# Layr-Labs/rust-kzg-bn254

Measured on AMD Instinct MI355X. Metric: G1-MSM (scalar,point) pairs/s = 2^20 x KZG coeff-form commitments/s, 2^20-point SRS, higher is better.
Workload: dtype int32x9 (29-bit limbs, 64-bit accumulate); 1 GPU; G1 MSM 2^20 scalars (KZG::commit_coeff_form), scalars resident in HBM; step k commits buffer k mod 8 (8 distinct resident scalar sets, 256 MiB); pipeline_depth=2, steps_per_launch=1

## Files before the change

### rust-kzg-bn254_amd/csrc/curve.h

```cpp
#pragma once
#include "field29.h"

#if !defined(__HIPCC__)
struct uint4 { uint32_t x, y, z, w; };
#endif

#if !defined(KZG_NO_MADD_PAIRED) && !defined(KZG_MADD_PAIRED)
#define KZG_MADD_PAIRED 1
#endif

namespace kzg {

struct Affine {
    Fq x, y;
};

struct Xyzz {
    Fq x, y, zz, zzz;
    bool inf;
};

KZG_HD void xyzz_set_inf(Xyzz& r) {
    fe_set_zero(r.x); fe_set_zero(r.y); fe_set_zero(r.zz); fe_set_zero(r.zzz);
    r.inf = true;
// ... 12 lines not shown
    Fq u, v, w, s, m, t, xx;
    fe_dbl(u, y2); fe_norm(u);
    fe_sqr(v, u);
    fe_mul(w, u, v);
    fe_mul(s, x2, v);
    fe_sqr(xx, x2);
    fe_add(m, xx, xx); fe_add(m, m, xx); fe_norm(m);
    fe_sqr(r.x, m);
    fe_sub(r.x, r.x, s); fe_sub(r.x, r.x, s); fe_norm(r.x);
    fe_sub(t, s, r.x);
    fe_mul(t, m, t);
    fe_mul(u, w, y2);
    fe_sub(r.y, t, u); fe_norm(r.y);
    r.zz = v;
    r.zzz = w;
    r.inf = false;
}

KZG_HD_NOINLINE void xyzz_dbl_affine(Xyzz& r, const Fq& x2, const Fq& y2) { xyzz_dbl_affine_impl(r, x2, y2); }

KZG_HD void xyzz_dbl_impl(Xyzz& r, const Xyzz& p) {
    if (p.inf) { r = p; return; }
    Fq u, v, w, s, m, t, xx;
    fe_dbl(u, p.y); fe_norm(u);
    fe_sqr(v, u);
    fe_mul(w, u, v);
    fe_mul(s, p.x, v);
    fe_sqr(xx, p.x);
    fe_add(m, xx, xx); fe_add(m, m, xx); fe_norm(m);
    Fq x3, y3;
    fe_sqr(x3, m);
    fe_sub(x3, x3, s); fe_sub(x3, x3, s); fe_norm(x3);
    fe_sub(t, s, x3);
    fe_mul(t, m, t);
    fe_mul(u, w, p.y);
    fe_sub(y3, t, u); fe_norm(y3);
    fe_mul(r.zz, v, p.zz);
    fe_mul(r.zzz, w, p.zzz);
    r.x = x3; r.y = y3; r.inf = false;
}

KZG_HD_NOINLINE void xyzz_dbl(Xyzz& r, const Xyzz& p) { xyzz_dbl_impl(r, p); }

template <bool INLINE_SLOW>
KZG_HD void xyzz_madd_exceptional(Xyzz& acc, const Fq& x2, const Fq& y2s, const Fq& rr) {
    if (fe_is_zero_mod(rr)) {
        if (INLINE_SLOW) xyzz_dbl_affine_impl(acc, x2, y2s);
        else xyzz_dbl_affine(acc, x2, y2s);
    } else {
        xyzz_set_inf(acc);
    }
}

template <bool INLINE_SLOW = false>
KZG_HD void xyzz_madd(Xyzz& acc, const Affine& p, uint32_t neg) {
    if (acc.inf) { xyzz_from_affine(acc, p, neg); return; }
    Fq y2s, u2, s2, pp_, rr_, P, R, ppp, q, t, v;
    fe_cneg(y2s, p.y, neg);
#if defined(KZG_MADD_PAIRED)
    fe_mul2(u2, p.x, acc.zz, s2, y2s, acc.zzz);
#else
    fe_mul(u2, p.x, acc.zz);
    fe_mul(s2, y2s, acc.zzz);
#endif
    fe_sub(P, u2, acc.x);
    fe_sub(R, s2, acc.y);
#if defined(KZG_MADD_PAIRED)
    fe_sqr2(pp_, P, rr_, R);
#else
    fe_sqr(pp_, P);
    fe_sqr(rr_, R);
#endif
    if (__builtin_expect(fe_is_zero_mod(pp_), 0)) { xyzz_madd_exceptional<INLINE_SLOW>(acc, p.x, y2s, rr_); return; }
#if defined(KZG_MADD_PAIRED)
    fe_mul2(ppp, P, pp_, q, acc.x, pp_);
#else
    fe_mul(ppp, P, pp_);
    fe_mul(q, acc.x, pp_);
#endif
    fe_sub(v, rr_, ppp); fe_sub(v, v, q); fe_sub(v, v, q); fe_norm(v);
    fe_sub(t, q, v);
    fe_mulsub(acc.y, R, t, acc.y, ppp);
    acc.x = v;
#if defined(KZG_MADD_PAIRED)
    { Fq z2, z3; fe_mul2(z2, acc.zz, pp_, z3, acc.zzz, ppp); acc.zz = z2; acc.zzz = z3; }
#else
    fe_mul(acc.zz, acc.zz, pp_);
    fe_mul(acc.zzz, acc.zzz, ppp);
#endif
}

template <bool INLINE_SLOW>
KZG_HD void xyzz_add_exceptional(Xyzz& r, const Xyzz& a, const Fq& rr) {
    if (fe_is_zero_mod(rr)) {
        if (INLINE_SLOW) xyzz_dbl_impl(r, a);
        else xyzz_dbl(r, a);
    } else {
        xyzz_set_inf(r);
    }
}

template <bool INLINE_SLOW = false>
KZG_HD void xyzz_add(Xyzz& r, const Xyzz& a, const Xyzz& b) {
    if (a.inf) { r = b; return; }
    if (b.inf) { r = a; return; }
    Fq u1, u2, s1, s2, P, R, pp_, rr_, ppp, q, t, v;
    fe_mul(u1, a.x, b.zz);
    fe_mul(u2, b.x, a.zz);
    fe_mul(s1, a.y, b.zzz);
    fe_mul(s2, b.y, a.zzz);
    fe_sub(P, u2, u1);
    fe_sub(R, s2, s1);
    fe_sqr(pp_, P);
    fe_sqr(rr_, R);
    if (__builtin_expect(fe_is_zero_mod(pp_), 0)) { xyzz_add_exceptional<INLINE_SLOW>(r, a, rr_); return; }
    fe_mul(ppp, P, pp_);
    fe_mul(q, u1, pp_);
    fe_sub(v, rr_, ppp); fe_sub(v, v, q); fe_sub(v, v, q); fe_norm(v);
    fe_sub(t, q, v);
    Fq y3;
    fe_mulsub(y3, R, t, s1, ppp);
    fe_mul(t, a.zz, b.zz);
    fe_mul(r.zz, t, pp_);
    fe_mul(t, a.zzz, b.zzz);
    fe_mul(r.zzz, t, ppp);
    r.x = v; r.y = y3; r.inf = false;
}

KZG_HD bool affine_load(Affine& p, const uint4* __restrict__ src) {
    uint4 a = src[0], b = src[1], c = src[2], d = src[3];
    uint32_t wx[8] = {a.x, a.y, a.z, a.w, b.x, b.y, b.z, b.w};
    uint32_t wy[8] = {c.x, c.y, c.z, c.w, d.x, d.y, d.z, d.w};
    fe_unpack(p.x, wx);
    fe_unpack(p.y, wy);
    uint32_t any = a.x | a.y | a.z | a.w | b.x | b.y | b.z | b.w | c.x | c.y | c.z | c.w | d.x | d.y | d.z | d.w;
    return any != 0;
}

KZG_HD void xyzz_store(int32_t* __restrict__ base, size_t stride, size_t i, const Xyzz& v) {
    const Fq* c[4] = {&v.x, &v.y, &v.zz, &v.zzz};
#pragma unroll
    for (int q = 0; q < 4; ++q)
#pragma unroll
        for (int j = 0; j < NL; ++j) base[(size_t)(q * NL + j) * stride + i] = v.inf ? 0 : c[q]->l[j];
}
KZG_HD void xyzz_load(Xyzz& v, const int32_t* __restrict__ base, size_t stride, size_t i) {
    Fq* c[4] = {&v.x, &v.y, &v.zz, &v.zzz};
#pragma unroll
    for (int q = 0; q < 4; ++q)
#pragma unroll
        for (int j = 0; j < NL; ++j) c[q]->l[j] = base[(size_t)(q * NL + j) * stride + i];
    v.inf = fe_is_literal_zero(v.zz);
}

KZG_HD void affine_wire_to_device(uint32_t out[16], const uint32_t in[16]) {
    Fq x, y;
    fe_from_wire(x, in);
    fe_from_wire(y, in + 8);
    fe_canon(x);
    fe_canon(y);
    fe_pack(out, x);
    fe_pack(out + 8, y);
}
KZG_HD void xyzz_to_wire(uint32_t out[32], const Xyzz& v) {
    if (v.inf) {
#pragma unroll
        for (int j = 0; j < 32; ++j) out[j] = 0;
        return;
    }
    fe_to_wire(out, v.x);
    fe_to_wire(out + 8, v.y);
    fe_to_wire(out + 16, v.zz);
    fe_to_wire(out + 24, v.zzz);
}

}
```

### rust-kzg-bn254_amd/csrc/engine.h

```cpp
#pragma once
#include <hip/hip_runtime.h>
#include <cstdint>
#include <functional>
#include <map>
#include <mutex>
#include <string>
#include "../../include/kzg_bn254_mi355x.h"

namespace kzg {

struct DeviceBuffer {
    void* p = nullptr;
    size_t bytes = 0;
    hipError_t reserve(size_t need) {
        if (need <= bytes) return hipSuccess;
        if (p) { hipError_t e = hipFree(p); p = nullptr; bytes = 0; if (e != hipSuccess) return e; }
        size_t cap = need + need / 8;
        hipError_t e = hipMalloc(&p, cap);
        if (e == hipSuccess) bytes = cap;
        return e;
    }
    void release() { if (p) { (void)hipFree(p); p = nullptr; bytes = 0; } }
    template <class T> T* as() const { return reinterpret_cast<T*>(p); }
};
// ... 58 lines not shown
#endif

struct kzg_ctx {
    int device = 0;
    hipStream_t stream = nullptr;
    std::mutex mu;
    std::string last_error;
    int msm_c_override = 0;
    int msm_seg_override = 0;
    int reduction_lanes = 0;
    bool profiling = false;
    bool lds_attr_set = false;
    bool poly_lds_attr_set = false;
    uint32_t acc_wave_slots = 3 * 1024;
    kzg::MsmWorkspace msm;
    kzg::MsmWorkspace msm_x[KZG_NUM_SLOTS - 1];
    hipStream_t stream_x[KZG_NUM_SLOTS - 1] = {};
    kzg::MsmPending* slot_pending[KZG_NUM_SLOTS] = {};
    kzg::NttWorkspace ntt;
    int32_t* ondomain_inv[13] = {};
    kzg::NttWorkspace ntt_x[KZG_NUM_SLOTS - 1];
    void* vb_pinned = nullptr;
    size_t vb_pinned_bytes = 0;
    kzg::DeviceBuffer rccl_buf;
    void* rccl_pinned = nullptr;
    size_t rccl_pinned_bytes = 0;
    kzg::PolySet poly[KZG_NUM_SLOTS];
    kzg::LagProof lag[KZG_NUM_SLOTS];
    hipStream_t lag_stream = nullptr;
    hipEvent_t lag_phase1[KZG_NUM_SLOTS] = {};
    hipEvent_t lag_uploaded[KZG_NUM_SLOTS] = {};
    kzg::MsmWorkspace& slot_msm(int slot) { return slot ? msm_x[slot - 1] : msm; }
    kzg::BlobStream* blob_stream = nullptr;
    hipEvent_t last_sorted = nullptr;
    hipStream_t last_sorted_stream = nullptr;
    kzg::NttWorkspace& slot_ntt(int slot) { return slot ? ntt_x[slot - 1] : ntt; }
    kzg::DeviceBuffer mp[6];
    kzg::NttWorkspace mp_ntt;
    kzg::DeviceBuffer mv[4];
    kzg::NttWorkspace mv_ntt;
};

struct kzg_srs {
    kzg_ctx* ctx = nullptr;
    mutable std::mutex lazy_mu;
    uint4* d_points = nullptr;
    size_t n = 0;
    int pre_c = 0;
    int pre_W = 0;
    uint4* d_small = nullptr;
    int small_c = 0;
    int small_W = 0;
    uint4* d_bits = nullptr;
    mutable uint4* d_t3 = nullptr;
    mutable uint32_t t3_n = 0;
    std::map<size_t, kzg_srs*> lagrange;
    size_t lagrange_of = 0;
    std::map<std::pair<size_t, size_t>, uint4*> multiproof;
};

namespace kzg {

struct MsmBases {
    const uint4* points = nullptr;
    uint32_t table_stride = 0;
    int c = 0;
    int W = 0;
    bool bitsum = false;
    bool naf = false;
};
constexpr int SRS_SMALL_C = 15;
constexpr size_t SRS_SMALL_MAX = (size_t)1 << 13;
constexpr size_t SRS_NAF_MIN = (size_t)1 << 11;
constexpr size_t MSM_NAF_MIN = (size_t)1 << 14;
inline int srs_naf_c(size_t n) {
    if (n < ((size_t)1 << 15)) return 13;
    return n >= ((size_t)1 << 20) ? 17 : n >= ((size_t)1 << 18) ? 16 : 15;
}
inline uint4* srs_bits(const kzg_srs* srs) { std::lock_guard<std::mutex> lk(srs->lazy_mu); return srs->d_bits; }
inline uint4* srs_t3(const kzg_srs* srs) { std::lock_guard<std::mutex> lk(srs->lazy_mu); return srs->d_t3; }
inline kzg_srs* srs_cached_lagrange(const kzg_srs* srs, size_t n) {
    std::lock_guard<std::mutex> lk(srs->lazy_mu);
    auto it = srs->lagrange.find(n);
    return it == srs->lagrange.end() ? nullptr : it->second;
}
inline MsmBases srs_bases(const kzg_srs* srs, size_t offset, size_t n, bool allow_tables) {
    MsmBases b;
    std::lock_guard<std::mutex> lk(srs->lazy_mu);
    b.points = srs->d_points + 4 * offset;
    if (allow_tables && srs->pre_W > 0) {
        b.table_stride = (uint32_t)srs->n; b.c = srs->pre_c; b.W = srs->pre_W;
        if (srs->d_small && n <= SRS_SMALL_MAX) { b.points = srs->d_small + 4 * offset; b.c = srs->small_c; b.W = srs->small_W; }
        if (srs->d_bits && n <= 4096) {
            b.points = srs->d_bits + 4 * offset; b.c = 0; b.W = 255; b.bitsum = true;
        }
        if (srs->d_bits && n >= MSM_NAF_MIN) {
            b.points = srs->d_bits + 4 * offset; b.c = srs_naf_c(n); b.W = 255; b.naf = true;
        }
    }
    return b;
}

int32_t msm_run(kzg_ctx* ctx, const MsmBases& bases, const void* d_scalars, size_t n,
                uint64_t out_xy[8], uint8_t* out_inf, uint64_t* out_xyzz);

int32_t msm_slot_stream(kzg_ctx* ctx, int slot, hipStream_t* out);
int32_t msm_begin(kzg_ctx* ctx, int slot, const MsmBases& bases, const void* d_scalars, size_t n);
int32_t msm_end(kzg_ctx* ctx, int slot, uint64_t out_xy[8], uint8_t* out_inf, uint64_t* out_xyzz);
void msm_drop_slots(kzg_ctx* ctx);
int32_t msm_run_batch(kzg_ctx* ctx, const uint4* d_points, const void* d_scalars, size_t n, uint32_t batch,
                      uint64_t* out_xy, uint8_t* out_inf);

int32_t srs_precompute(kzg_ctx* ctx, kzg_srs* srs);
int32_t srs_build_bit_tables(kzg_ctx* ctx, kzg_srs* srs, bool force);
size_t msm_batch_capacity(size_t n);
int32_t msm_begin_batch(kzg_ctx* ctx, int slot, const MsmBases& bases, const void* const* d_scalars, size_t n, size_t count);
int32_t msm_end_batch(kzg_ctx* ctx, int slot, size_t count, uint64_t* out_xy, uint8_t* out_inf, uint64_t* out_xyzz);
int32_t msm_run_batch_tables(kzg_ctx* ctx, const MsmBases& bases, const void* d_scalars, size_t n, size_t polys, uint64_t* out_xy, uint8_t* out_inf);

int32_t points_wire_to_device(kzg_ctx* ctx, const uint4* d_wire, uint4* d_out, size_t n, uint32_t* d_off_curve_flag = nullptr);

struct NttTables {
    int32_t* lo = nullptr;
    int32_t* hi = nullptr;
    uint32_t lo_len = 0, hi_len = 0;
    int lo_bits = 0;
};
int32_t ntt_get_tables(kzg_ctx* ctx, int log_n, bool inverse, NttTables* out);

int32_t ntt_run(kzg_ctx* ctx, void* d_data, size_t n, bool inverse, hipStream_t st = nullptr, NttWorkspace* ws = nullptr);

int32_t srs_generate(kzg_ctx* ctx, const uint64_t tau_mont[4], uint64_t first_power, size_t n, uint4* d_points);
int32_t srs_download(kzg_ctx* ctx, const uint4* d_points, size_t n, uint64_t* out_xy);
int32_t srs_decompress(kzg_ctx* ctx, const uint8_t* bytes, size_t n, uint4* d_points, uint32_t* err_kind, uint32_t* err_index, bool ark_le = false);

int32_t g1_ifft_run(kzg_ctx* ctx, const kzg_srs* srs, size_t n, uint64_t* out_xy);
int32_t g1_ifft_device(kzg_ctx* ctx, const kzg_srs* srs, size_t n, uint4* d_out, bool wire);
int32_t g1_fft_planes(kzg_ctx* ctx, hipStream_t st, const int32_t* in, size_t in_stride, size_t n, int32_t* out, int32_t* tmp, bool inverse, bool scaled);
int32_t g1fft_planes_to_affine(kzg_ctx* ctx, hipStream_t st, const int32_t* planes, size_t n, uint4* d_out, bool wire, int32_t* scratch);
int32_t multiproof_cache(kzg_ctx* ctx, kzg_srs* srs, size_t n, size_t l, const uint4** out);
int32_t multiproof_run(kzg_ctx* ctx, kzg_srs* srs, const uint64_t* poly_mont, size_t n, bool eval_form, size_t l, uint64_t* out_xy, uint8_t* out_inf);
void multiproof_drop(kzg_srs* srs);
// ... 52 lines not shown
```

### rust-kzg-bn254_amd/csrc/msm.hip

```cpp
#include "engine.h"
#include <new>
#include "msm_kernels.h"
#include "host_curve.h"
#include "host_pairing.h"

#include <algorithm>
#include <cstdlib>
#include <chrono>
#include <cstdio>
#include <cstring>
#include <vector>

namespace kzg {

constexpr uint32_t MSM_BATCH_POLYS_MAX = 1024;
constexpr uint32_t MSM_MAX_OUT = 16384;
constexpr size_t SORT1_MAX_LDS = 131072;

void MsmWorkspace::release() {
    DeviceBuffer* all[] = {&scalars, &bases, &bases_wire, &digits, &sorted, &count, &blockbase, &sort_tmp, &sort_key, &sort_small, &offs, &block_sums,
                           &head, &cont, &blob, &bucket, &chunkS, &chunkTmp, &chunkA, &out_wire};
    for (auto* b : all) b->release();
    if (pinned_out) { (void)hipHostFree(pinned_out); pinned_out = nullptr; }
    if (ev_ready) { for (auto& e : ev) (void)hipEventDestroy(e); ev_ready = false; }
// ... 336 lines not shown
                           ws.count.as<uint32_t>(), ws.blockbase.as<uint32_t>(), (const uint8_t*)nullptr);
        hipLaunchKernelGGL(k_sort2_bin<false>, dim3(p.Hb), dim3(SORT2_BIN_THREADS), 0, st, ws.sort_tmp.as<uint32_t>(), cstart, p.Hb, ws.count.as<uint32_t>(),
                           d_offs, ws.sorted.as<uint32_t>(), (const uint32_t*)bin_cap, (const uint8_t*)nullptr);
        hipLaunchKernelGGL(k_sort2_scatter2<false>, dim3(p.tiles2cap), dim3(256), 0, st, ws.sort_tmp.as<uint32_t>(), cstart, tstart, tile_bin, p.Hb,
                           d_offs, ws.blockbase.as<uint32_t>(), ws.sorted.as<uint32_t>(), (const uint8_t*)nullptr);
        }
        KZG_MARK(3);
    } else if (lean_sort) {
        if (clean_g < p.G) KZG_HIP_TRY(ctx, hipMemsetAsync(ws.count.p, 0, (size_t)p.G * 4, st));
        hipLaunchKernelGGL(k_msm_digits, dim3(gn), dim3(256), 0, st, d_scalars, n_total, p.n, p.c, p.W, ws.digits.as<uint32_t>(), ws.count.as<uint32_t>());
        KZG_MARK(1);
        hipLaunchKernelGGL(k_scan_counts_1wg<true>, dim3(1), dim3(SCAN1_THREADS), 0, st, ws.count.as<uint32_t>(), p.G, d_offs, ws.blockbase.as<uint32_t>());
        KZG_MARK(2);
        const uint32_t ge = (uint32_t)((entries + 255) / 256);
        hipLaunchKernelGGL(k_sort_small_scatter, dim3(ge), dim3(256), 0, st, ws.digits.as<uint32_t>(), (uint32_t)entries, p.n, p.set_len, p.B,
                           d_offs, ws.blockbase.as<uint32_t>(), p.idx_stride, (uint32_t)p.W, ws.sorted.as<uint32_t>(), 1);
        KZG_MARK(3);
        ws.count_zero_ptr = ws.count.p;
        ws.count_zero_g = p.G;
    } else {
        KZG_HIP_TRY(ctx, hipMemsetAsync(ws.count.p, 0, (size_t)p.G * 4, st));
        hipLaunchKernelGGL(k_msm_digits, dim3(gn), dim3(256), 0, st, d_scalars, n_total, p.n, p.c, p.W, ws.digits.as<uint32_t>(), (uint32_t*)nullptr);
        KZG_MARK(1);
        if (p.sort_small) {
            const uint32_t ge = (uint32_t)((entries + 255) / 256);
            KZG_HIP_TRY(ctx, hipMemsetAsync(ws.blockbase.p, 0, (size_t)p.G * 4, st));
            hipLaunchKernelGGL(k_sort_small_hist, dim3(ge), dim3(256), 0, st, ws.digits.as<uint32_t>(), (uint32_t)entries, p.set_len, p.B,
                               ws.count.as<uint32_t>());
            scan_counts();
            KZG_MARK(2);
            hipLaunchKernelGGL(k_sort_small_scatter, dim3(ge), dim3(256), 0, st, ws.digits.as<uint32_t>(), (uint32_t)entries, p.n, p.set_len, p.B,
                               d_offs, ws.blockbase.as<uint32_t>(), p.idx_stride, (uint32_t)p.W, ws.sorted.as<uint32_t>());
        } else {
            hipLaunchKernelGGL(k_sort_hist, dim3(p.tiles), dim3(256), lds_bytes, st, ws.digits.as<uint32_t>(), p.set_len, p.tile_len,
                               p.tiles_per_set, p.B, ws.count.as<uint32_t>(), ws.blockbase.as<uint32_t>());
            scan_counts();
            KZG_MARK(2);
            hipLaunchKernelGGL(k_sort_scatter, dim3(p.tiles), dim3(256), lds_bytes, st, ws.digits.as<uint32_t>(), p.n, p.set_len, p.tile_len,
                               p.tiles_per_set, p.B, d_offs, ws.blockbase.as<uint32_t>(), p.idx_stride,
                               (uint32_t)p.W, ws.sorted.as<uint32_t>());
        }
        KZG_MARK(3);
    }
    KZG_MARK(4);
    if (p.tables) {
        if (!ws.ev_sorted) KZG_HIP_TRY(ctx, hipEventCreateWithFlags(&ws.ev_sorted, hipEventDisableTiming));
        KZG_HIP_TRY(ctx, hipEventRecord(ws.ev_sorted, st));
        ctx->last_sorted = ws.ev_sorted;
        ctx->last_sorted_stream = st;
    }
    phases.begin("kzg:msm:accumulate");
    const bool fused = p.tables && !p.naf && (double)entries <= 2.5 * (double)p.B;
    p.fused = fused;
    if (!fused)
        hipLaunchKernelGGL(k_msm_accumulate, dim3(p.nl / 256), dim3(256), 0, st, bases.points, ws.sorted.as<uint32_t>(), d_offs, p.G,
                           ws.head.as<int32_t>(), (size_t)p.G, ws.cont.as<int32_t>(), (size_t)p.nl, p.idx_log, p.stride_adj);
    KZG_MARK(5);
    phases.begin("kzg:msm:bucket reduction");
    uint32_t n_out;
    if (p.tables) {
        if (fused && p.quad)
            hipLaunchKernelGGL(k_msm_bucket_bits1q_fused, dim3(G1), dim3(256), 0, st, bases.points, ws.sorted.as<uint32_t>(), d_offs, p.B, p.idx_log,
                               p.stride_adj, G1, ws.chunkS.as<int32_t>(), (size_t)7 * G1, d_out);
        else if (fused)
            hipLaunchKernelGGL(k_msm_bucket_bits1p_fused, dim3(G1), dim3(128), 0, st, bases.points, ws.sorted.as<uint32_t>(), d_offs, p.B, p.idx_log,
                               p.stride_adj, G1, ws.chunkS.as<int32_t>(), (size_t)7 * G1, d_out);
        else if (p.quad && (G1 <= 512 || ctx->reduction_lanes == 4))
            hipLaunchKernelGGL(k_msm_bucket_bits1q, dim3(G1), dim3(256), 0, st, d_offs, p.B, p.nl, ws.head.as<int32_t>(), (size_t)p.G,
                               ws.cont.as<int32_t>(), (size_t)p.nl, G1, ws.chunkS.as<int32_t>(), (size_t)7 * G1, d_out);
        else
            hipLaunchKernelGGL(k_msm_bucket_bits1p, dim3(G1), dim3(128), 0, st, d_offs, p.B, p.nl, ws.head.as<int32_t>(), (size_t)p.G,
                               ws.cont.as<int32_t>(), (size_t)p.nl, G1, ws.chunkS.as<int32_t>(), (size_t)7 * G1, d_out);
        KZG_MARK(6);
        if (p.polys && p.c == 7) {
            hipLaunchKernelGGL(k_batch_finish, dim3((p.polys + 63) / 64), dim3(64), 0, st, ws.chunkS.as<int32_t>(), (size_t)7 * G1, G1, d_out);
            n_out = p.polys;
        } else if (G1 == 1) {
            n_out = 7;
        } else {
            const uint32_t waves2 = 7 * G1p;
            if (p.quad)
                hipLaunchKernelGGL(k_red_bits2q, dim3(waves2), dim3(256), 0, st, ws.chunkS.as<int32_t>(), (size_t)7 * G1, G1, G1p, d_out);
            else
                hipLaunchKernelGGL(k_red_bits2p, dim3((waves2 + 1) / 2), dim3(128), 0, st, ws.chunkS.as<int32_t>(), (size_t)7 * G1, G1, G1p, d_out);
            n_out = 13 * G1p;
        }
    } else {
        const uint32_t gg = (p.G + 255) / 256;
        hipLaunchKernelGGL(k_msm_bucket_fin, dim3(gg), dim3(256), 0, st, d_offs, p.G, p.nl, p.m, n_chunks, ws.head.as<int32_t>(), (size_t)p.G,
                           ws.cont.as<int32_t>(), (size_t)p.nl, ws.bucket.as<int32_t>(), (size_t)p.G);
        const uint32_t gc = (n_chunks + 255) / 256;
        KZG_MARK(6);
        hipLaunchKernelGGL(k_red_chunk_sums, dim3(gc), dim3(256), 0, st, ws.bucket.as<int32_t>(), (size_t)p.G, n_chunks, p.m,
                           ws.chunkS.as<int32_t>(), (size_t)n_chunks);
        hipLaunchKernelGGL(k_red_suffix_scan, dim3(n_windows), dim3(p.T), 0, st, ws.chunkS.as<int32_t>(), ws.chunkTmp.as<int32_t>(),
                           (size_t)n_chunks, p.T);
        hipLaunchKernelGGL(k_red_chunk_running, dim3(gc), dim3(256), 0, st, ws.bucket.as<int32_t>(), (size_t)p.G,
                           ws.chunkS.as<int32_t>(), (size_t)n_chunks, n_chunks, p.T, p.m, ws.chunkA.as<int32_t>());
        hipLaunchKernelGGL(k_red_window_sum, dim3(n_windows), dim3(p.T), 0, st, ws.chunkA.as<int32_t>(), (size_t)n_chunks, p.T,
                           d_out);
        n_out = n_windows;
    }
    KZG_MARK(7);
    phases.end();
    KZG_HIP_TRY(ctx, hipGetLastError());
    if (n_out > out_cap || out_off + n_out > MSM_MAX_OUT) {
        (void)hipStreamSynchronize(st);
        ctx->last_error = "MSM result points exceed this launch's window of the result buffer";
// ... 302 lines not shown
            ctx->last_error = "a kzg_*_begin is still in flight: the batched commitments use the slots' streams and workspaces themselves";
            return KZG_ERR_INVALID_ARG;
        }
    const int cb = batch_bucket_bits(n);
    const size_t per = std::min<size_t>(std::min<size_t>(MSM_BATCH_POLYS_MAX, (size_t)65536 >> (cb - 1)), MSM_MAX_LAUNCH / n);
    if (per == 0) return KZG_ERR_TOO_LARGE;
    constexpr int DEPTH = 3;
    static_assert(DEPTH <= KZG_NUM_SLOTS, "one slot per launch in flight");
    Pending pend[DEPTH];
    size_t first[DEPTH] = {}, cnt[DEPTH] = {};
    bool busy[DEPTH] = {};
    static thread_local std::vector<kzg_host::Xyzz> res;
    res.resize(std::min(per, polys));
    const uint4* sc = reinterpret_cast<const uint4*>(d_scalars);
    auto collect = [&](int s) -> int32_t {
        hipStream_t st = nullptr;
        (void)msm_slot_stream(ctx, s, &st);
        int32_t rc = msm_finish(ctx, ctx->slot_msm(s), st, pend[s], res.data());
        busy[s] = false;
        if (rc != KZG_OK) return rc;
        kzg_host::xyzz_batch_to_affine(res.data(), cnt[s], out_xy + 8 * first[s]);
        if (out_inf)
            for (size_t i = 0; i < cnt[s]; ++i) {
                const uint64_t* q = out_xy + 8 * (first[s] + i);
                out_inf[first[s] + i] = (q[0] | q[1] | q[2] | q[3] | q[4] | q[5] | q[6] | q[7]) == 0 ? 1 : 0;
            }
        return KZG_OK;
    };
    int32_t rc = KZG_OK;
    size_t launch = 0;
    for (size_t done = 0; done < polys && rc == KZG_OK; done += per, ++launch) {
        const int s = (int)(launch % DEPTH);
        if (busy[s]) rc = collect(s);
        if (rc != KZG_OK) break;
        const size_t k = std::min(per, polys - done);
        hipStream_t st = nullptr;
        rc = msm_slot_stream(ctx, s, &st);
        if (rc != KZG_OK) break;
        rc = msm_enqueue(ctx, ctx->slot_msm(s), st, bases, sc + 2 * done * n, n * k, 1, &pend[s], 0, MSM_MAX_OUT, (uint32_t)k);
        if (rc != KZG_OK) break;
        first[s] = done; cnt[s] = k; busy[s] = true;
    }
    for (size_t q = 0; q < DEPTH; ++q) {
        const int s = (int)((launch + q) % DEPTH);
        if (!busy[s]) continue;
        const int32_t r2 = collect(s);
        if (rc == KZG_OK) rc = r2;
    }
    return rc;
}

}

#if defined(KZG_DEVICE_BOUND_CHECK)
#include "field29.h"
KZG_BOUND_CHECK_EXPORTS(msm)
#endif
```

### rust-kzg-bn254_amd/csrc/msm_kernels.h

```cpp
#pragma once
#include <hip/hip_runtime.h>
#include "curve_pair.h"
#include "curve_quad.h"
#include "naf.h"

namespace kzg {

__device__ __forceinline__ void latency_bound_kernel() {
#if !defined(KZG_NO_SETPRIO)
    __builtin_amdgcn_s_setprio(3);
#endif
}

constexpr uint32_t DIGIT_NONE = 0xFFFFFFFFu;
constexpr int RED_T = 512;

__global__ void __launch_bounds__(256)
k_msm_digits(const uint4* __restrict__ scalars, uint32_t n_total, uint32_t n, int c, int W, uint32_t* __restrict__ digits,
             uint32_t* __restrict__ count = nullptr ) {
    latency_bound_kernel();
    uint32_t j = blockIdx.x * blockDim.x + threadIdx.x;
    if (j >= n_total) return;
    const uint32_t msm = j / n, i = j - msm * n;
    uint4 lo = scalars[2 * (size_t)j], hi = scalars[2 * (size_t)j + 1];
// ... 576 lines not shown
        __syncthreads();
        if (t < 64) {
            const uint32_t c0 = hist[2 * t], c1 = hist[2 * t + 1];
            uint32_t incl = c0 + c1;
            for (int d = 1; d < 64; d <<= 1) { const uint32_t x = __shfl_up(incl, d, 64); if ((int)t >= d) incl += x; }
            lstart[2 * t] = incl - (c0 + c1); lstart[2 * t + 1] = incl - c1;
        }
        __syncthreads();
#pragma unroll
        for (int j = 0; j < SORT2_BIN_PER; ++j)
            if (j * SORT2_BIN_THREADS + t < cn) {
                const uint32_t slot = lstart[kq[j]] + r[j];
                buf[slot] = v[j];
                if (NAF) bufk[slot] = (uint8_t)kq[j];
            }
        __syncthreads();
        for (uint32_t i = t; i < cn; i += SORT2_BIN_THREADS) {
            const uint32_t x = buf[i], k = NAF ? (uint32_t)bufk[i] : (x >> SORT2_IDX_BITS) & (SORT2_LO - 1);
            sorted[gpos[k] + (i - lstart[k])] = NAF ? x : x & (0x80000000u | SORT2_IDX_MASK);
        }
        __syncthreads();
        if (t < SORT2_LO) gpos[t] += hist[t];
    }
}

#ifndef KZG_RUN_SERIAL
#define KZG_RUN_SERIAL 8
#endif
constexpr uint32_t RUN_SERIAL = KZG_RUN_SERIAL;
constexpr uint32_t NP_SERIAL = 10;

__device__ __forceinline__ void xyzz_shfl_down(Xyzz& r, const Xyzz& v, int d) {
    const Fq* s[4] = {&v.x, &v.y, &v.zz, &v.zzz};
    Fq* t[4] = {&r.x, &r.y, &r.zz, &r.zzz};
#pragma unroll
    for (int q = 0; q < 4; ++q)
#pragma unroll
        for (int j = 0; j < NL; ++j) t[q]->l[j] = __shfl_down(s[q]->l[j], d, 64);
    r.inf = __shfl_down((int)v.inf, d, 64) != 0;
}
__device__ __forceinline__ uint32_t acc_seg_len(uint32_t E, uint32_t nl) { return (E + nl - 1) / nl; }

#ifdef KZG_ACC_NOGATHER
#define KZG_ACC_IDX(v) ((v) & 0xFFu)
#else
#define KZG_ACC_IDX(v) ((v) & 0x7FFFFFFFu)
#endif
__device__ __forceinline__ size_t acc_point_index(uint32_t ix, uint32_t idx_log, uint32_t stride_adj) {
    return (size_t)ix + (size_t)(ix >> idx_log) * stride_adj;
}
#ifndef KZG_ACC_WAVES
#define KZG_ACC_WAVES 3
#endif
__global__ void __launch_bounds__(256) __attribute__((amdgpu_waves_per_eu(KZG_ACC_WAVES, KZG_ACC_WAVES)))
k_msm_accumulate(const uint4* __restrict__ points, const uint32_t* __restrict__ sorted, const uint32_t* __restrict__ offs, uint32_t G,
                 int32_t* __restrict__ head, size_t head_stride, int32_t* __restrict__ cont, size_t cont_stride,
                 uint32_t idx_log, uint32_t stride_adj) {
    const uint32_t nl = gridDim.x * blockDim.x;
    const uint32_t t = blockIdx.x * blockDim.x + threadIdx.x;
    const uint32_t lane = threadIdx.x & 63;
#ifdef KZG_ACC_STAMPS
    unsigned long long* stamps = reinterpret_cast<unsigned long long*>(cont + cont_stride * 36) + 8 * (size_t)(t >> 6);
    const unsigned long long stamp0 = __builtin_amdgcn_s_memrealtime();
    unsigned long long flush_ticks = 0, flush_events = 0, stamp_loop = 0;
#endif
    const uint32_t E = offs[G];
    const uint32_t L = acc_seg_len(E, nl);
    const unsigned long long b64 = (unsigned long long)t * L;
    const uint32_t begin = b64 < E ? (uint32_t)b64 : E;
    const uint32_t end = (b64 + L < E) ? (uint32_t)(b64 + L) : E;
    const bool active = begin < end;
    uint32_t g = 0, next = 0, g0 = 0xFFFFFFFFu;
    bool is_cont = false, long_run = false;
    if (active) {
        uint32_t lo = 0, hi = G;
#ifdef KZG_ACC_BINARY_SEARCH
        while (hi - lo > 1) {
            const uint32_t mid = (lo + hi) >> 1;
            if (offs[mid] <= begin) lo = mid; else hi = mid;
        }
#else
        while (hi - lo > 1) {
            const uint32_t s = (hi - lo + 15) >> 4;
            uint32_t cnt = 0;
#pragma unroll
            for (uint32_t j = 1; j < 16; ++j) {
                const uint32_t p = lo + j * s;
                const uint32_t v = p < hi ? offs[p] : 0xFFFFFFFFu;
                cnt += v <= begin ? 1u : 0u;
            }
            const uint32_t nlo = lo + cnt * s, nhi = lo + (cnt + 1) * s;
            if (cnt < 15 && nhi < hi) hi = nhi;
            lo = nlo;
        }
#endif
        g = lo;
        const uint32_t o0 = offs[g];
        next = offs[g + 1];
        is_cont = o0 < begin;
        if (is_cont) { long_run = ((next - 1) / L - o0 / L) > RUN_SERIAL; g0 = g; }
    }
    __shared__ int32_t park[4 * NL * 256];
    const uint32_t tl = threadIdx.x;
    bool parked = false, parked_cont = false;
    uint32_t park_g = 0;
    bool cont_in_regs = false;
    Xyzz acc;
    xyzz_set_inf(acc);
    uint32_t next2 = 0;
    if (active) next2 = offs[g + 2 <= G ? g + 2 : G];
    auto flush = [&](bool more) {
        const bool as_cont = is_cont && g == g0;
        if (more && !parked) {
            const Fq* c4[4] = {&acc.x, &acc.y, &acc.zz, &acc.zzz};
#pragma unroll
            for (int q = 0; q < 4; ++q)
#pragma unroll
                for (int j = 0; j < NL; ++j) park[(q * NL + j) * 256 + tl] = acc.inf ? 0 : c4[q]->l[j];
            parked = true; parked_cont = as_cont; park_g = g;
        } else if (!as_cont) {
            xyzz_store(head, head_stride, g, acc);
        } else if (!long_run || more) {
            xyzz_store(cont, cont_stride, t, acc);
        } else {
            cont_in_regs = true;
        }
    };
#ifdef KZG_ACC_STAMPS
    stamp_loop = __builtin_amdgcn_s_memrealtime();
#endif
    if (active) {
        const uint32_t last = end - 1;
        uint32_t v = sorted[begin];
        uint32_t v1 = sorted[begin + 1 < end ? begin + 1 : last];
        const uint4* src = points + 4 * acc_point_index(KZG_ACC_IDX(v), idx_log, stride_adj);
        uint4 q0 = src[0], q1 = src[1], q2 = src[2], q3 = src[3];
        for (uint32_t e = begin; e < end; ++e) {
#ifdef KZG_ACC_STAMPS
            const bool any_cross = __any(e == next);
            unsigned long long f0 = 0;
            if (any_cross) f0 = __builtin_amdgcn_s_memrealtime();
#endif
            if (__builtin_expect(e == next, 0)) {
                flush(true);
                xyzz_set_inf(acc);
                ++g; next = next2;
                while (next == e) { ++g; next = offs[g + 1]; }
                next2 = offs[g + 2 <= G ? g + 2 : G];
            }
#ifdef KZG_ACC_STAMPS
            if (any_cross) { flush_ticks += __builtin_amdgcn_s_memrealtime() - f0; flush_events += 1; }
#endif
            const uint32_t neg = v >> 31;
            uint32_t wx[8] = {q0.x, q0.y, q0.z, q0.w, q1.x, q1.y, q1.z, q1.w};
            uint32_t wy[8] = {q2.x, q2.y, q2.z, q2.w, q3.x, q3.y, q3.z, q3.w};
            const uint32_t any = q0.x | q0.y | q0.z | q0.w | q1.x | q1.y | q1.z | q1.w | q2.x | q2.y | q2.z | q2.w | q3.x | q3.y | q3.z | q3.w;
            Affine p;
            fe_unpack(p.x, wx);
            fe_unpack(p.y, wy);
            v = v1;
            src = points + 4 * acc_point_index(KZG_ACC_IDX(v), idx_log, stride_adj);
            q0 = src[0]; q1 = src[1]; q2 = src[2]; q3 = src[3];
            v1 = sorted[e + 2 < end ? e + 2 : last];
            if (any == 0) continue;
            xyzz_madd<true>(acc, p, neg);
        }
        flush(false);
    }
    const bool in_scan = active && is_cont && long_run;
    Xyzz c;
    xyzz_set_inf(c);
    if (cont_in_regs) c = acc;
    if (parked) {
        Xyzz v;
        Fq* c4[4] = {&v.x, &v.y, &v.zz, &v.zzz};
#pragma unroll
        for (int q = 0; q < 4; ++q)
#pragma unroll
            for (int j = 0; j < NL; ++j) c4[q]->l[j] = park[(q * NL + j) * 256 + tl];
        v.inf = fe_is_literal_zero(v.zz);
        if (!parked_cont) xyzz_store(head, head_stride, park_g, v);
        else if (!long_run) xyzz_store(cont, cont_stride, t, v);
        else c = v;
    }
#ifdef KZG_ACC_STAMPS
    if (lane == 0) {
        unsigned int hwid, xcc;
        asm volatile("s_getreg_b32 %0, hwreg(HW_REG_HW_ID)" : "=s"(hwid));
        asm volatile("s_getreg_b32 %0, hwreg(HW_REG_XCC_ID)" : "=s"(xcc));
        stamps[0] = stamp0; stamps[1] = __builtin_amdgcn_s_memrealtime(); stamps[2] = hwid; stamps[3] = xcc;
        stamps[4] = flush_ticks; stamps[5] = flush_events; stamps[6] = stamp_loop;
    }
#endif
    if (!__any(in_scan)) return;
    const uint32_t key = in_scan ? g0 : 0xFFFFFFFFu;
#pragma unroll 1
    for (int d = 1; d < 64; d <<= 1) {
        const uint32_t kd = __shfl_down(key, d, 64);
        const bool join = in_scan && (lane + d < 64) && kd == key;
        if (!__any(join)) continue;
        Xyzz u;
        xyzz_shfl_down(u, c, d);
        if (join) {
            Xyzz r;
            xyzz_add<true>(r, c, u);
            c = r;
        }
    }
    const uint32_t kprev = __shfl_up(key, 1, 64);
    if (in_scan && (lane == 0 || kprev != key)) xyzz_store(cont, cont_stride, t, c);
}

__device__ __forceinline__ size_t bucket_pos(uint32_t g, uint32_t m, uint32_t n_chunks) {
    return (size_t)(g % m) * n_chunks + (g / m);
}
struct BucketSpan {
    uint32_t g, t1, np;
    bool long_run;
// ... 801 lines not shown
```

### rust-kzg-bn254_amd/csrc/srs.hip

```cpp
#include "engine.h"
#include "curve.h"
#include "fe_invert.h"

#include <cstdlib>

namespace kzg {

template <class F>
__device__ __forceinline__ void fe_inverse(Fe<F>& out, const Fe<F>& a) {
#if !defined(KZG_INVERT_FERMAT)
    fe_inverse_safegcd(out, a);
#else
    Fe<F> acc, base = a;
    fe_set_one(acc);
    uint32_t e[8];
#pragma unroll
    for (int j = 0; j < 8; ++j) e[j] = F::P32[j];
    e[0] -= 2u;
    for (int w = 0; w < 8; ++w) {
        uint32_t bits = e[w];
        for (int b = 0; b < 32; ++b) {
            if (w == 7 && b >= 30) break;
            if (bits & 1u) fe_mul(acc, acc, base);
            fe_sqr(base, base);
// ... 237 lines not shown
            err = 2;
        } else {
            Fq one_plain, yc;
            fe_set_zero(one_plain);
            one_plain.l[0] = 1;
            fe_mul(yc, y, one_plain);
            fe_canon(yc);
            uint32_t yw[8];
            fe_pack(yw, yc);
            bool ge = true;
            for (int k = 7; k >= 0; --k) {
                if (yw[k] != FqParams::HALF_UP32[k]) { ge = yw[k] > FqParams::HALF_UP32[k]; break; }
            }
            const bool negate = ge ? (flag == FLAG_SMALLEST) : (flag == FLAG_LARGEST);
            Fq ys;
            fe_canon(y);
            fe_cneg(ys, y, negate ? 1u : 0u);
            fe_norm(ys);
            fe_canon(x);
            fe_canon(ys);
            fe_pack(o, x);
            fe_pack(o + 8, ys);
        }
    }
    if (err) {
        if (atomicCAS(&status[0], 0u, err) == 0u) status[1] = i;
    }
    out[4 * (size_t)i] = make_uint4(o[0], o[1], o[2], o[3]);
    out[4 * (size_t)i + 1] = make_uint4(o[4], o[5], o[6], o[7]);
    out[4 * (size_t)i + 2] = make_uint4(o[8], o[9], o[10], o[11]);
    out[4 * (size_t)i + 3] = make_uint4(o[12], o[13], o[14], o[15]);
}

__global__ void __launch_bounds__(256)
k_points_device_to_wire(const uint4* __restrict__ in, uint4* __restrict__ out, size_t n) {
    size_t i = (size_t)blockIdx.x * blockDim.x + threadIdx.x;
    if (i >= n) return;
    Affine p;
    bool ok = affine_load(p, in + 4 * i);
    uint32_t o[16];
    if (!ok) {
#pragma unroll
        for (int j = 0; j < 16; ++j) o[j] = 0;
    } else {
        fe_to_wire(o, p.x);
        fe_to_wire(o + 8, p.y);
    }
    out[4 * i] = make_uint4(o[0], o[1], o[2], o[3]);
    out[4 * i + 1] = make_uint4(o[4], o[5], o[6], o[7]);
    out[4 * i + 2] = make_uint4(o[8], o[9], o[10], o[11]);
    out[4 * i + 3] = make_uint4(o[12], o[13], o[14], o[15]);
}

int32_t srs_generate(kzg_ctx* ctx, const uint64_t tau[4], uint64_t first_power, size_t n, uint4* d_points) {
    if (n == 0) return KZG_OK;
    KZG_HIP_TRY(ctx, ctx->poly[0].a.reserve(n * 32 + 64));
    KZG_HIP_TRY(ctx, ctx->poly[0].small.reserve(4096));
    uint4* d_tau = ctx->poly[0].small.as<uint4>();
    KZG_HIP_TRY(ctx, hipMemcpyAsync(d_tau, tau, 32, hipMemcpyHostToDevice, ctx->stream));
    const uint32_t per = 64;
    uint32_t lanes = (uint32_t)((n + per - 1) / per);
    hipLaunchKernelGGL(k_fr_powers, dim3((lanes + 255) / 256), dim3(256), 0, ctx->stream, d_tau, ctx->poly[0].a.as<uint4>(), first_power, (uint32_t)n, per);
    hipLaunchKernelGGL(k_srs_powers, dim3((unsigned)((n + 255) / 256)), dim3(256), 0, ctx->stream, ctx->poly[0].a.as<uint4>(), d_points, (uint32_t)n);
    KZG_HIP_TRY(ctx, hipGetLastError());
    KZG_HIP_TRY(ctx, hipStreamSynchronize(ctx->stream));
    return KZG_OK;
}

int32_t srs_precompute(kzg_ctx* ctx, kzg_srs* srs) {
    if (opt_no_precompute()) return KZG_OK;
    const size_t n = srs->n;
    if (n < 128) return KZG_OK;
    int lg = 0;
    while ((n >> (lg + 1)) != 0) ++lg;
    int c = 13;
    if (lg >= 14) c = 15;
    if (lg >= 18) c = 17;
    auto build = [&](int cw, uint4** out, int* out_W) -> int32_t {
        *out = nullptr;
        const int W = (255 + cw - 1) / cw;
        const size_t bytes = (size_t)W * n * 64;
        if (bytes > ((size_t)48 << 30) || (size_t)W * n >= ((size_t)1 << 31)) return KZG_OK;
        uint4* table = nullptr;
        hipError_t e = hipMalloc(reinterpret_cast<void**>(&table), bytes);
        if (e != hipSuccess) { (void)hipGetLastError(); return KZG_OK; }
        e = hipMemcpyAsync(table, srs->d_points, n * 64, hipMemcpyDeviceToDevice, ctx->stream);
        for (int w = 1; w < W && e == hipSuccess; ++w) {
            hipLaunchKernelGGL(k_srs_window_step, dim3((unsigned)((n + 255) / 256)), dim3(256), 0, ctx->stream,
                               table + 4 * (size_t)(w - 1) * n, table + 4 * (size_t)w * n, n, cw);
        }
        if (e == hipSuccess) e = hipGetLastError();
        if (e == hipSuccess) e = hipStreamSynchronize(ctx->stream);
        if (e != hipSuccess) { (void)hipFree(table); return set_error(ctx, e, "building the SRS window tables"); }
        *out = table; *out_W = W;
        return KZG_OK;
    };
    uint4* table = nullptr;
    int W = 0;
    { int32_t rc = build(c, &table, &W); if (rc != KZG_OK) return rc; }
    if (!table) return KZG_OK;
    if (c > SRS_SMALL_C) {
        uint4* t2 = nullptr; int W2 = 0;
        int32_t rc = build(SRS_SMALL_C, &t2, &W2);
        if (rc != KZG_OK) { (void)hipFree(table); return rc; }
        if (t2) { srs->d_small = t2; srs->small_c = SRS_SMALL_C; srs->small_W = W2; }
    }
    KZG_HIP_TRY(ctx, hipFree(srs->d_points));
    srs->d_points = table;
    srs->pre_c = c;
    srs->pre_W = W;
    return srs_build_bit_tables(ctx, srs, false);
}

int32_t srs_build_bit_tables(kzg_ctx* ctx, kzg_srs* srs, bool force) {
    if (opt_no_naf()) return KZG_OK;
    const size_t n = srs->n;
    std::lock_guard<std::mutex> lazy(srs->lazy_mu);
    if (n == 0 || (n < SRS_NAF_MIN && !force) || n > ((size_t)1 << 22) || srs->d_bits) return KZG_OK;
    const size_t bytes = (size_t)255 * n * 64;
    size_t free_b = 0, total_b = 0;
    if (hipMemGetInfo(&free_b, &total_b) != hipSuccess) { (void)hipGetLastError(); return KZG_OK; }
    if (bytes + (bytes >> 2) + ((size_t)8 << 30) > free_b) return KZG_OK;
    uint4* bits = nullptr;
    if (hipMalloc(reinterpret_cast<void**>(&bits), bytes) != hipSuccess) { (void)hipGetLastError(); return KZG_OK; }
// ... 54 lines not shown
```

Before: 950.1 million pairs/s.

## Drop per-add exceptional checks in bucket accumulation, replay buckets on detected degeneracy

```diff
diff --git a/rust-kzg-bn254_amd/csrc/curve.h b/rust-kzg-bn254_amd/csrc/curve.h
--- a/rust-kzg-bn254_amd/csrc/curve.h
+++ b/rust-kzg-bn254_amd/csrc/curve.h
@@ -88,7 +88,7 @@
     }
 }
 
-template <bool INLINE_SLOW = false>
+template <bool INLINE_SLOW = false, bool CHECKED = true>
 KZG_HD void xyzz_madd(Xyzz& acc, const Affine& p, uint32_t neg) {
     if (acc.inf) { xyzz_from_affine(acc, p, neg); return; }
     Fq y2s, u2, s2, pp_, rr_, P, R, ppp, q, t, v;
@@ -107,7 +107,7 @@
     fe_sqr(pp_, P);
     fe_sqr(rr_, R);
 #endif
-    if (__builtin_expect(fe_is_zero_mod(pp_), 0)) { xyzz_madd_exceptional<INLINE_SLOW>(acc, p.x, y2s, rr_); return; }
+    if (CHECKED && __builtin_expect(fe_is_zero_mod(pp_), 0)) { xyzz_madd_exceptional<INLINE_SLOW>(acc, p.x, y2s, rr_); return; }
 #if defined(KZG_MADD_PAIRED)
     fe_mul2(ppp, P, pp_, q, acc.x, pp_);
 #else
@@ -180,6 +180,13 @@
 #pragma unroll
         for (int j = 0; j < NL; ++j) base[(size_t)(q * NL + j) * stride + i] = v.inf ? 0 : c[q]->l[j];
 }
+KZG_HD void xyzz_store_zeroed(int32_t* __restrict__ base, size_t stride, size_t i, const Xyzz& v) {
+    const Fq* c[4] = {&v.x, &v.y, &v.zz, &v.zzz};
+#pragma unroll
+    for (int q = 0; q < 4; ++q)
+#pragma unroll
+        for (int j = 0; j < NL; ++j) base[(size_t)(q * NL + j) * stride + i] = c[q]->l[j];
+}
 KZG_HD void xyzz_load(Xyzz& v, const int32_t* __restrict__ base, size_t stride, size_t i) {
     Fq* c[4] = {&v.x, &v.y, &v.zz, &v.zzz};
 #pragma unroll
diff --git a/rust-kzg-bn254_amd/csrc/engine.h b/rust-kzg-bn254_amd/csrc/engine.h
--- a/rust-kzg-bn254_amd/csrc/engine.h
+++ b/rust-kzg-bn254_amd/csrc/engine.h
@@ -134,6 +134,7 @@
     int small_c = 0;
     int small_W = 0;
     uint4* d_bits = nullptr;
+    bool identity_free = false;
     mutable uint4* d_t3 = nullptr;
     mutable uint32_t t3_n = 0;
     std::map<size_t, kzg_srs*> lagrange;
@@ -150,6 +151,7 @@
     int W = 0;
     bool bitsum = false;
     bool naf = false;
+    bool identity_free = false;
 };
 constexpr int SRS_SMALL_C = 15;
 constexpr size_t SRS_SMALL_MAX = (size_t)1 << 13;
@@ -170,6 +172,7 @@
     MsmBases b;
     std::lock_guard<std::mutex> lk(srs->lazy_mu);
     b.points = srs->d_points + 4 * offset;
+    b.identity_free = srs->identity_free;
     if (allow_tables && srs->pre_W > 0) {
         b.table_stride = (uint32_t)srs->n; b.c = srs->pre_c; b.W = srs->pre_W;
         if (srs->d_small && n <= SRS_SMALL_MAX) { b.points = srs->d_small + 4 * offset; b.c = srs->small_c; b.W = srs->small_W; }
diff --git a/rust-kzg-bn254_amd/csrc/msm.hip b/rust-kzg-bn254_amd/csrc/msm.hip
--- a/rust-kzg-bn254_amd/csrc/msm.hip
+++ b/rust-kzg-bn254_amd/csrc/msm.hip
@@ -412,8 +412,11 @@
     phases.begin("kzg:msm:accumulate");
     const bool fused = p.tables && !p.naf && (double)entries <= 2.5 * (double)p.B;
     p.fused = fused;
-    if (!fused)
-        hipLaunchKernelGGL(k_msm_accumulate, dim3(p.nl / 256), dim3(256), 0, st, bases.points, ws.sorted.as<uint32_t>(), d_offs, p.G,
+    if (!fused && bases.identity_free)
+        hipLaunchKernelGGL(k_msm_accumulate<false>, dim3(p.nl / 256), dim3(256), 0, st, bases.points, ws.sorted.as<uint32_t>(), d_offs, p.G,
+                           ws.head.as<int32_t>(), (size_t)p.G, ws.cont.as<int32_t>(), (size_t)p.nl, p.idx_log, p.stride_adj);
+    else if (!fused)
+        hipLaunchKernelGGL(k_msm_accumulate<true>, dim3(p.nl / 256), dim3(256), 0, st, bases.points, ws.sorted.as<uint32_t>(), d_offs, p.G,
                            ws.head.as<int32_t>(), (size_t)p.G, ws.cont.as<int32_t>(), (size_t)p.nl, p.idx_log, p.stride_adj);
     KZG_MARK(5);
     phases.begin("kzg:msm:bucket reduction");
@@ -822,6 +825,15 @@
 
 }
 
+#if defined(KZG_TEST_HOOKS)
+extern "C" int kzg_test_acc_replays(unsigned long long* out, int reset) {
+    if (out && hipMemcpyFromSymbol(out, HIP_SYMBOL(kzg::g_acc_replays), sizeof(unsigned long long)) != hipSuccess) return -1;
+    const unsigned long long zero = 0;
+    if (reset && hipMemcpyToSymbol(HIP_SYMBOL(kzg::g_acc_replays), &zero, sizeof(zero)) != hipSuccess) return -1;
+    return 0;
+}
+#endif
+
 #if defined(KZG_DEVICE_BOUND_CHECK)
 #include "field29.h"
 KZG_BOUND_CHECK_EXPORTS(msm)
diff --git a/rust-kzg-bn254_amd/csrc/msm_kernels.h b/rust-kzg-bn254_amd/csrc/msm_kernels.h
--- a/rust-kzg-bn254_amd/csrc/msm_kernels.h
+++ b/rust-kzg-bn254_amd/csrc/msm_kernels.h
@@ -652,6 +652,25 @@
 #ifndef KZG_ACC_WAVES
 #define KZG_ACC_WAVES 3
 #endif
+#ifdef KZG_TEST_HOOKS
+__device__ unsigned long long g_acc_replays;
+#endif
+__device__ __noinline__ Xyzz acc_replay(const uint4* __restrict__ points, const uint32_t* __restrict__ sorted, uint32_t lo, uint32_t hi, uint32_t idx_log, uint32_t stride_adj) {
+    Xyzz r;
+    xyzz_set_inf(r);
+#pragma unroll 1
+    for (uint32_t e = lo; e < hi; ++e) {
+        const uint32_t v = sorted[e];
+        Affine p;
+        if (!affine_load(p, points + 4 * acc_point_index(KZG_ACC_IDX(v), idx_log, stride_adj))) continue;
+        xyzz_madd<true>(r, p, v >> 31);
+    }
+#ifdef KZG_TEST_HOOKS
+    atomicAdd(&g_acc_replays, 1ull);
+#endif
+    return r;
+}
+template <bool IDENTITY_BASES>
 __global__ void __launch_bounds__(256) __attribute__((amdgpu_waves_per_eu(KZG_ACC_WAVES, KZG_ACC_WAVES)))
 k_msm_accumulate(const uint4* __restrict__ points, const uint32_t* __restrict__ sorted, const uint32_t* __restrict__ offs, uint32_t G,
                  int32_t* __restrict__ head, size_t head_stride, int32_t* __restrict__ cont, size_t cont_stride,
@@ -710,18 +729,24 @@
     uint32_t next2 = 0;
     if (active) next2 = offs[g + 2 <= G ? g + 2 : G];
     auto flush = [&](bool more) {
+        if (__builtin_expect(!acc.inf && fe_is_zero_mod(acc.zz), 0)) {
+            const uint32_t o0 = offs[g], o1 = offs[g + 1];
+            acc = acc_replay(points, sorted, o0 > begin ? o0 : begin, o1 < end ? o1 : end, idx_log, stride_adj);
+        }
+        KZG_REQUIRE(!acc.inf || (fe_is_literal_zero(acc.x) && fe_is_literal_zero(acc.y) && fe_is_literal_zero(acc.zz) && fe_is_literal_zero(acc.zzz)),
+                    KZG_SITE_IS_ZERO_MOD, "k_msm_accumulate: inf without zero limbs", acc.zz);
         const bool as_cont = is_cont && g == g0;
         if (more && !parked) {
             const Fq* c4[4] = {&acc.x, &acc.y, &acc.zz, &acc.zzz};
 #pragma unroll
             for (int q = 0; q < 4; ++q)
 #pragma unroll
-                for (int j = 0; j < NL; ++j) park[(q * NL + j) * 256 + tl] = acc.inf ? 0 : c4[q]->l[j];
+                for (int j = 0; j < NL; ++j) park[(q * NL + j) * 256 + tl] = c4[q]->l[j];
             parked = true; parked_cont = as_cont; park_g = g;
         } else if (!as_cont) {
-            xyzz_store(head, head_stride, g, acc);
+            xyzz_store_zeroed(head, head_stride, g, acc);
         } else if (!long_run || more) {
-            xyzz_store(cont, cont_stride, t, acc);
+            xyzz_store_zeroed(cont, cont_stride, t, acc);
         } else {
             cont_in_regs = true;
         }
@@ -733,8 +758,10 @@
         const uint32_t last = end - 1;
         uint32_t v = sorted[begin];
         uint32_t v1 = sorted[begin + 1 < end ? begin + 1 : last];
-        const uint4* src = points + 4 * acc_point_index(KZG_ACC_IDX(v), idx_log, stride_adj);
-        uint4 q0 = src[0], q1 = src[1], q2 = src[2], q3 = src[3];
+        typedef uint32_t u32x4 __attribute__((ext_vector_type(4)));
+        const u32x4* const pts = reinterpret_cast<const u32x4*>(points);
+        const u32x4* src = pts + 4 * acc_point_index(KZG_ACC_IDX(v), idx_log, stride_adj);
+        u32x4 q0 = src[0], q1 = src[1], q2 = src[2], q3 = src[3];
         for (uint32_t e = begin; e < end; ++e) {
 #ifdef KZG_ACC_STAMPS
             const bool any_cross = __any(e == next);
@@ -752,6 +779,7 @@
             if (any_cross) { flush_ticks += __builtin_amdgcn_s_memrealtime() - f0; flush_events += 1; }
 #endif
             const uint32_t neg = v >> 31;
+            asm("" : "+v"(q0), "+v"(q1), "+v"(q2), "+v"(q3));
             uint32_t wx[8] = {q0.x, q0.y, q0.z, q0.w, q1.x, q1.y, q1.z, q1.w};
             uint32_t wy[8] = {q2.x, q2.y, q2.z, q2.w, q3.x, q3.y, q3.z, q3.w};
             const uint32_t any = q0.x | q0.y | q0.z | q0.w | q1.x | q1.y | q1.z | q1.w | q2.x | q2.y | q2.z | q2.w | q3.x | q3.y | q3.z | q3.w;
@@ -759,11 +787,11 @@
             fe_unpack(p.x, wx);
             fe_unpack(p.y, wy);
             v = v1;
-            src = points + 4 * acc_point_index(KZG_ACC_IDX(v), idx_log, stride_adj);
+            src = pts + 4 * acc_point_index(KZG_ACC_IDX(v), idx_log, stride_adj);
             q0 = src[0]; q1 = src[1]; q2 = src[2]; q3 = src[3];
             v1 = sorted[e + 2 < end ? e + 2 : last];
-            if (any == 0) continue;
-            xyzz_madd<true>(acc, p, neg);
+            if (IDENTITY_BASES && any == 0) continue;
+            xyzz_madd<true, false>(acc, p, neg);
         }
         flush(false);
     }
diff --git a/rust-kzg-bn254_amd/csrc/srs.hip b/rust-kzg-bn254_amd/csrc/srs.hip
--- a/rust-kzg-bn254_amd/csrc/srs.hip
+++ b/rust-kzg-bn254_amd/csrc/srs.hip
@@ -313,6 +313,15 @@
     out[4 * i + 3] = make_uint4(o[12], o[13], o[14], o[15]);
 }
 
+__global__ void __launch_bounds__(256)
+k_srs_count_identity(const uint4* __restrict__ in, size_t n, uint32_t* __restrict__ count) {
+    const size_t i = (size_t)blockIdx.x * blockDim.x + threadIdx.x;
+    if (i >= n) return;
+    const uint4 a = in[4 * i], b = in[4 * i + 1], c = in[4 * i + 2], d = in[4 * i + 3];
+    const uint32_t any = a.x | a.y | a.z | a.w | b.x | b.y | b.z | b.w | c.x | c.y | c.z | c.w | d.x | d.y | d.z | d.w;
+    if (any == 0) atomicAdd(count, 1u);
+}
+
 int32_t srs_generate(kzg_ctx* ctx, const uint64_t tau[4], uint64_t first_power, size_t n, uint4* d_points) {
     if (n == 0) return KZG_OK;
     KZG_HIP_TRY(ctx, ctx->poly[0].a.reserve(n * 32 + 64));
@@ -329,8 +338,23 @@
 }
 
 int32_t srs_precompute(kzg_ctx* ctx, kzg_srs* srs) {
+    const size_t n = srs->n;
+    if (n) {
+        uint32_t* d_count = nullptr;
+        uint32_t identities = 1;
+        KZG_HIP_TRY(ctx, hipMalloc(reinterpret_cast<void**>(&d_count), 4));
+        hipError_t e = hipMemsetAsync(d_count, 0, 4, ctx->stream);
+        if (e == hipSuccess) {
+            hipLaunchKernelGGL(k_srs_count_identity, dim3((unsigned)((n + 255) / 256)), dim3(256), 0, ctx->stream, srs->d_points, n, d_count);
+            e = hipGetLastError();
+        }
+        if (e == hipSuccess) e = hipMemcpyAsync(&identities, d_count, 4, hipMemcpyDeviceToHost, ctx->stream);
+        if (e == hipSuccess) e = hipStreamSynchronize(ctx->stream);
+        (void)hipFree(d_count);
+        if (e != hipSuccess) return set_error(ctx, e, "counting the identity points of the SRS");
+        srs->identity_free = identities == 0;
+    }
     if (opt_no_precompute()) return KZG_OK;
-    const size_t n = srs->n;
     if (n < 128) return KZG_OK;
     int lg = 0;
     while ((n >> (lg + 1)) != 0) ++lg;
```

Result: faster. 968.2 million pairs/s, median of 6 (+1.9%).
